# k2-fsa/Flow2GAN

Measured on AMD Instinct MI355X. Metric: audio-seconds/sec (train step, G+D fwd/bwd) mel_24k_base, higher is better.
Workload: dtype f32 (fp32-class products on the bf16 matrix pipe for the long reductions and the direct MRD convs: every fp32 operand as three bf16 pieces = 24 significand bits, the six v_mfma_f32_32x32x16_bf16 products with i + j <= 2 per fp32 product, fp32 accumulate, error <= 2^-23 per product; short reductions ; 1 GPU; mel_24k_base GAN stage-2 train step: D-step + G-step, each on its own batch (MPD+MRD+FM+multi-scale mel), fwd+bwd+grad all-reduce, no optimizer (metric is fwd/bwd); per_gpu_batch=64, gan=gan_multi_scale_mel_recon, parallelism=dp1, optimizer=none

## Files before the change

flow2gan_amd/csrc/conv32x6.hip:

```cpp
#include <stdlib.h>

#include "common.h"


namespace {

typedef float f32x16 __attribute__((ext_vector_type(16)));
typedef float f32x4 __attribute__((ext_vector_type(4)));
typedef __bf16 bf16x8 __attribute__((ext_vector_type(8)));
typedef unsigned int u32x2 __attribute__((ext_vector_type(2)));
typedef unsigned int u32x4 __attribute__((ext_vector_type(4)));

constexpr int C = 32, KH = 3, KW = 9, NTAP = KH * KW;
constexpr int PB = 208;

__device__ __attribute__((aligned(16))) float c6_zero[4] = {0.f, 0.f, 0.f, 0.f};

__device__ __forceinline__ void split3(const f32x4 v, u32x2& p0, u32x2& p1, u32x2& p2) {
  unsigned a0, a1, a2, b0, b1, b2;
  f2g_split3_pair(v.x, v.y, a0, a1, a2);
  f2g_split3_pair(v.z, v.w, b0, b1, b2);
  p0 = u32x2{a0, b0};
  p1 = u32x2{a1, b1};
  p2 = u32x2{a2, b2};
}

__device__ __forceinline__ void store_px3(unsigned char* p, const f32x4 v) {
  u32x2 p0, p1, p2;
  split3(v, p0, p1, p2);
  *reinterpret_cast<u32x2*>(p) = p0;
  *reinterpret_cast<u32x2*>(p + 64) = p1;
  *reinterpret_cast<u32x2*>(p + 128) = p2;
}

struct frag6 {
  bf16x8 v[2][3];
};
__device__ __forceinline__ void ld6(frag6& f, const unsigned char* p) {
#pragma unroll
  for (int ks = 0; ks < 2; ++ks)
#pragma unroll
    for (int q = 0; q < 3; ++q) f.v[ks][q] = *reinterpret_cast<const bf16x8*>(p + q * 64 + ks * 32);
}
__device__ __forceinline__ void mm6(const frag6& a, const frag6& b, f32x16& acc0, f32x16& acc1) {
#define F2G_X6_PAIR(I, J)                                                               \
  acc0 = __builtin_amdgcn_mfma_f32_32x32x16_bf16(a.v[0][I], b.v[0][J], acc0, 0, 0, 0);   \
  acc1 = __builtin_amdgcn_mfma_f32_32x32x16_bf16(a.v[1][I], b.v[1][J], acc1, 0, 0, 0);
  F2G_X6_PAIR(2, 0) F2G_X6_PAIR(1, 1) F2G_X6_PAIR(0, 2) F2G_X6_PAIR(1, 0) F2G_X6_PAIR(0, 1) F2G_X6_PAIR(0, 0)
#undef F2G_X6_PAIR
}
__device__ __forceinline__ void tap6(const unsigned char* Ab, const unsigned char* Bb, f32x16& acc0, f32x16& acc1) {
  frag6 a, b;
  ld6(a, Ab);
  ld6(b, Bb);
  mm6(a, b, acc0, acc1);
}

template <int D>
__device__ __forceinline__ int div_small(int x) {
  static_assert(D == 39 || D == 23 || D == 20 || D == 12, "magic constants below");
  return (x * (D == 39 ? 1681 : D == 23 ? 2850 : D == 20 ? 3277 : 5462)) >> 16;
}

template <int TW_>
__device__ __forceinline__ void px_of_row(int pg, int r, int& ph, int& pw) {
  if (TW_ == 16) {
    ph = 2 * pg + (r >> 4);
    pw = (r + 12 * (r >> 4)) & 15;
  } else {
    const int p = pg * 32 + r;
    ph = p / TW_;
    pw = p % TW_;
  }
}

template <int TH_, int TW_>
__global__ __launch_bounds__(512, 1) void conv32_s2_fwd6_kernel(const f2g_conv32_desc d, int tiles_w,
                                                               int tiles_h, int ntiles) {
  constexpr int IHv = TH_ + KH - 1, IWv = TW_ + (KW - 1) / 2, XW = 2 * IWv - 1;
  constexpr int SUBB = IHv * IWv * PB + 64;
  constexpr int NCHK = (IHv * XW * (C / 4) + 511) / 512;
  constexpr int PGB = (TW_ == 16 ? 2 : 4) * IWv * PB;
  constexpr int NKS = 2 * NTAP, KPW = 7;
  static_assert(TH_ * TW_ == 128, "a block owns 128 output pixels");
  static_assert(6 * KPW + 2 * (KPW - 1) == NKS, "the k split covers the reduction exactly");
  extern __shared__ __attribute__((aligned(16))) unsigned char smb[];
  unsigned char* At = smb;
  float* red = reinterpret_cast<float*>(smb + 2 * SUBB);
  const int tid = threadIdx.x, lane = tid & 63;
  const int wave = __builtin_amdgcn_readfirstlane(tid >> 6);
  const int li = lane & 31, hh = lane >> 5;
  const int c4 = tid & 7;
  const int px0 = tid >> 3;
  auto tile_pos = [&](int tile, int& sq, int& h0, int& w0) {
    const int tw = tile % tiles_w, rest = tile / tiles_w;
    const int th = rest % tiles_h;
    sq = rest / tiles_h;
    h0 = th * TH_;
    w0 = tw * TW_;
  };
  auto load_patch = [&](int tile, f32x4 (&pf)[NCHK]) {
    int sq, h0, w0;
    tile_pos(tile, sq, h0, w0);
    const int x0 = 2 * w0 - (KW - 1) / 2;
    const float* org = d.x + (long long)sq * d.x_seq + (long long)(h0 - 1) * d.x_line + (long long)x0 * C + c4 * 4;
    const int xl = (int)d.x_line;
    int pxb = px0;
    asm volatile("" : "+v"(pxb));
#pragma unroll
    for (int q = 0; q < NCHK; ++q) {
      const int px = pxb + 64 * q;
      const int r = div_small<XW>(px), xr = px - r * XW;
      const int h = h0 - 1 + r, x = x0 + xr;
      const bool ok = px < IHv * XW && h >= 0 && h < d.H && x >= 0 && x < d.Win;
      pf[q] = *reinterpret_cast<const f32x4*>(ok ? org + (r * xl + xr * C) : c6_zero);
    }
  };
  auto store_patch = [&](const f32x4 (&pf)[NCHK]) {
    int pxb = px0;
    asm volatile("" : "+v"(pxb));
#pragma unroll
    for (int q = 0; q < NCHK; ++q) {
      const int px = pxb + 64 * q;
      const int r = div_small<XW>(px), xr = px - r * XW;
      if (px < IHv * XW) store_px3(At + (xr & 1) * SUBB + (r * IWv + (xr >> 1)) * PB + c4 * 8, pf[q]);
    }
  };
  int tile = blockIdx.x;
  if (tile >= ntiles) return;
  f32x4 pf[NCHK];
  load_patch(tile, pf);
  const int k0 = wave * KPW - (wave == 7 ? 1 : 0);
  const bool seven = wave < 6;
  bf16x8 wf[KPW][3];
  int koff[KPW];
  {
    const unsigned char* wrow = reinterpret_cast<const unsigned char*>(d.w) + li * (NTAP * 192) + hh * 16;
#pragma unroll
    for (int j = 0; j < KPW; ++j) {
      int k = k0 + j;
      k = k < NKS ? k : NKS - 1;
      const int t = k >> 1, ks = k & 1;
      const int dh = t / KW, jw = t - dh * KW;
      koff[j] = (jw & 1) * SUBB + (dh * IWv + (jw >> 1)) * PB + ks * 32;
#pragma unroll
      for (int q = 0; q < 3; ++q) wf[j][q] = *reinterpret_cast<const bf16x8*>(wrow + t * 192 + q * 64 + ks * 32);
    }
  }
  int ph, pw;
  px_of_row<TW_>(0, li, ph, pw);
  const unsigned char* Ap = At + (ph * IWv + pw) * PB + hh * 16;
  const int orow = (wave & 3) * 8 + (lane >> 3), och = 4 * (lane & 7);
  f32x4 bias4 = {0.f, 0.f, 0.f, 0.f};
  if (d.bias) bias4 = f32x4{d.bias[och], d.bias[och + 1], d.bias[och + 2], d.bias[och + 3]};
  store_patch(pf);
  __syncthreads();
  for (; tile < ntiles; tile += gridDim.x) {
    const int nxt = tile + gridDim.x;
    const bool more = nxt < ntiles;
    load_patch(more ? nxt : tile, pf);
    f32x16 acc[4];
#pragma unroll
    for (int g4 = 0; g4 < 4; ++g4)
#pragma unroll
      for (int e = 0; e < 16; ++e) acc[g4][e] = 0.f;
    bf16x8 a[2][3];
#pragma unroll
    for (int q = 0; q < 3; ++q) a[0][q] = *reinterpret_cast<const bf16x8*>(Ap + koff[0] + q * 64);
#pragma unroll
    for (int u = 0; u < 4 * KPW; ++u) {
      const int j = u >> 2, g4 = u & 3;
      if (u + 1 < 4 * KPW) {
        const unsigned char* an = Ap + koff[(u + 1) >> 2] + ((u + 1) & 3) * PGB;
#pragma unroll
        for (int q = 0; q < 3; ++q) a[(u + 1) & 1][q] = *reinterpret_cast<const bf16x8*>(an + q * 64);
      }
      __builtin_amdgcn_sched_barrier(0);
      if (j < KPW - 1 || seven) {
#define F2G_X6_ONE(I, J) acc[g4] = __builtin_amdgcn_mfma_f32_32x32x16_bf16(a[u & 1][I], wf[j][J], acc[g4], 0, 0, 0);
        F2G_X6_ONE(2, 0) F2G_X6_ONE(1, 1) F2G_X6_ONE(0, 2) F2G_X6_ONE(1, 0) F2G_X6_ONE(0, 1) F2G_X6_ONE(0, 0)
#undef F2G_X6_ONE
      }
      __builtin_amdgcn_sched_barrier(0);
    }
    int sq, h0, w0;
    tile_pos(tile, sq, h0, w0);
    float* ys = d.y + (long long)sq * d.y_seq;
    __syncthreads();
#pragma unroll
    for (int p2 = 0; p2 < 2; ++p2) {
      if (p2) __syncthreads();
#pragma unroll
      for (int g2 = 0; g2 < 2; ++g2)
#pragma unroll
        for (int e = 0; e < 16; ++e)
          red[((wave * 2 + g2) * 32 + (e & 3) + 8 * (e >> 2) + 4 * hh) * 32 + li] = acc[2 * p2 + g2][e];
      __syncthreads();
      f32x4 s = *reinterpret_cast<const f32x4*>(red + (((wave >> 2)) * 32 + orow) * 32 + och);
#pragma unroll
      for (int w8 = 1; w8 < 8; ++w8) {
        const f32x4 v = *reinterpret_cast<const f32x4*>(red + ((w8 * 2 + (wave >> 2)) * 32 + orow) * 32 + och);
        s.x += v.x, s.y += v.y, s.z += v.z, s.w += v.w;
      }
      s.x += bias4.x, s.y += bias4.y, s.z += bias4.z, s.w += bias4.w;
      if (d.lrelu_slope != 0.f) {
        s.x = s.x > 0.f ? s.x : d.lrelu_slope * s.x;
        s.y = s.y > 0.f ? s.y : d.lrelu_slope * s.y;
        s.z = s.z > 0.f ? s.z : d.lrelu_slope * s.z;
        s.w = s.w > 0.f ? s.w : d.lrelu_slope * s.w;
      }
      int qh, qw;
      px_of_row<TW_>(2 * p2 + (wave >> 2), orow, qh, qw);
      const int oh = h0 + qh, ow = w0 + qw;
      if (oh < d.H && ow < d.Wout)
        *reinterpret_cast<f32x4*>(ys + (long long)oh * d.y_line + (long long)ow * C + och) = s;
      if (p2 == 0 && more) store_patch(pf);
    }
  }
}

template <int TH_, int TW_>
__global__ __launch_bounds__(512, 1) void conv32_s2_dgrad6_kernel(const f2g_conv32_desc d, int tiles_w,
                                                                 int tiles_h, int ntiles) {
  constexpr int IHv = TH_ + KH - 1, GWv = TW_ + 4;
  constexpr int NCHK = (IHv * GWv * (C / 4) + 511) / 512;
  constexpr int PGB = (TW_ == 16 ? 2 : 4) * GWv * PB;
  constexpr int KPW = 8;
  static_assert(TH_ * TW_ == 128, "a block owns 128 positions of each column parity");
  extern __shared__ __attribute__((aligned(16))) unsigned char smb[];
  unsigned char* At = smb;
  float* red = reinterpret_cast<float*>(smb + IHv * GWv * PB);
  const int tid = threadIdx.x, lane = tid & 63;
  const int wave = __builtin_amdgcn_readfirstlane(tid >> 6);
  const int li = lane & 31, hh = lane >> 5;
  const int wq = wave & 3, E = wave >> 2;
  const int c4 = tid & 7;
  const int NU = E ? 4 : 5;
  const int Wp = (d.Win + 1 - E) / 2;
  const int px0 = tid >> 3;
  auto tile_pos = [&](int tile, int& sq, int& h0, int& m0) {
    const int tw = tile % tiles_w, rest = tile / tiles_w;
    const int th = rest % tiles_h;
    sq = rest / tiles_h;
    h0 = th * TH_;
    m0 = tw * TW_;
  };
  auto load_patch = [&](int tile, f32x4 (&pf)[NCHK]) {
    int sq, h0, m0;
    tile_pos(tile, sq, h0, m0);
    const float* org = d.x + (long long)sq * d.x_seq + (long long)(h0 - 1) * d.x_line + (long long)(m0 - 2) * C + c4 * 4;
    const int xl = (int)d.x_line;
    int pxb = px0;
    asm volatile("" : "+v"(pxb));
#pragma unroll
    for (int q = 0; q < NCHK; ++q) {
      const int px = pxb + 64 * q;
      const int r = div_small<GWv>(px), xc = px - r * GWv;
      const int h = h0 - 1 + r, c = m0 - 2 + xc;
      const bool ok = px < IHv * GWv && h >= 0 && h < d.H && c >= 0 && c < d.Wout;
      pf[q] = *reinterpret_cast<const f32x4*>(ok ? org + (r * xl + xc * C) : c6_zero);
    }
  };
  auto store_patch = [&](const f32x4 (&pf)[NCHK]) {
#pragma unroll
    for (int q = 0; q < NCHK; ++q) {
      const int px = px0 + 64 * q;
      if (px < IHv * GWv) store_px3(At + px * PB + c4 * 8, pf[q]);
    }
  };
  int tile = blockIdx.x;
  if (tile >= ntiles) return;
  f32x4 pf[NCHK];
  load_patch(tile, pf);
  const int nk = E ? 6 : (wq < 2 ? 8 : 7);
  const int k0 = E ? 6 * wq : (wq < 2 ? 8 * wq : 16 + 7 * (wq - 2));
  bf16x8 wf[KPW][3];
  int koff[KPW];
  {
    const unsigned char* wrow = reinterpret_cast<const unsigned char*>(d.w) + li * 192 + hh * 16;
    const int nks = 2 * KH * NU;
#pragma unroll
    for (int j = 0; j < KPW; ++j) {
      int k = k0 + j;
      k = k < nks ? k : nks - 1;
      const int ti = k >> 1, ks = k & 1;
      const int dh = E ? ti >> 2 : (ti * 13) >> 6;
      const int u = ti - dh * NU;
      koff[j] = ks * 32 - (dh * GWv + u) * PB;
      const int tile_w = dh * KW + E + 2 * u;
#pragma unroll
      for (int q = 0; q < 3; ++q)
        wf[j][q] = *reinterpret_cast<const bf16x8*>(wrow + tile_w * (C * 192) + q * 64 + ks * 32);
    }
  }
  int ph, pw;
  px_of_row<TW_>(0, li, ph, pw);
  const unsigned char* Ap = At + ((ph + 2) * GWv + pw + 4) * PB + hh * 16;
  const int och = 4 * (lane & 7);
  const bool msk = d.mask_src != nullptr, fm = d.fm_ref != nullptr;
  const float fmw = fm ? d.fm_w * (d.fm_wdev ? d.fm_wdev[0] : 1.f) : 0.f;
  float cs[4] = {0.f, 0.f, 0.f, 0.f};
  store_patch(pf);
  __syncthreads();
  for (; tile < ntiles; tile += gridDim.x) {
    const int nxt = tile + gridDim.x;
    const bool more = nxt < ntiles;
    load_patch(more ? nxt : tile, pf);
    int sq, h0, m0;
    tile_pos(tile, sq, h0, m0);
    const long long tbase = (long long)sq * d.y_seq + (long long)h0 * d.y_line + (long long)(2 * m0 + E) * C;
    auto item_off = [&](int jj) {
      int qh, qw, l8 = lane >> 3;
      asm volatile("" : "+v"(l8));
      px_of_row<TW_>(2 * (jj >> 1) + (wq >> 1), (wq & 1) * 16 + l8 + 8 * (jj & 1), qh, qw);
      return (h0 + qh < d.H && m0 + qw < Wp) ? qh * (int)d.y_line + 2 * qw * C + och : -1;
    };
    f32x4 my[4];
    if (msk && !fm) {
#pragma unroll
      for (int jj = 0; jj < 4; ++jj) {
        const int o = item_off(jj);
        my[jj] = *reinterpret_cast<const f32x4*>(d.mask_src + (o >= 0 ? tbase + o : 0));
      }
    }
    f32x16 acc[4];
#pragma unroll
    for (int g4 = 0; g4 < 4; ++g4)
#pragma unroll
      for (int e = 0; e < 16; ++e) acc[g4][e] = 0.f;
    bf16x8 a[2][3];
#pragma unroll
    for (int q = 0; q < 3; ++q) a[0][q] = *reinterpret_cast<const bf16x8*>(Ap + koff[0] + q * 64);
#pragma unroll
    for (int u = 0; u < 4 * KPW; ++u) {
      const int j = u >> 2, g4 = u & 3;
      if (u + 1 < 4 * KPW) {
        const unsigned char* an = Ap + koff[(u + 1) >> 2] + ((u + 1) & 3) * PGB;
#pragma unroll
        for (int q = 0; q < 3; ++q) a[(u + 1) & 1][q] = *reinterpret_cast<const bf16x8*>(an + q * 64);
      }
      __builtin_amdgcn_sched_barrier(0);
      if (j < 6 || j < nk) {
#define F2G_X6_ONE(I, J) acc[g4] = __builtin_amdgcn_mfma_f32_32x32x16_bf16(a[u & 1][I], wf[j][J], acc[g4], 0, 0, 0);
        F2G_X6_ONE(2, 0) F2G_X6_ONE(1, 1) F2G_X6_ONE(0, 2) F2G_X6_ONE(1, 0) F2G_X6_ONE(0, 1) F2G_X6_ONE(0, 0)
#undef F2G_X6_ONE
      }
      __builtin_amdgcn_sched_barrier(0);
    }
    __syncthreads();
#pragma unroll
    for (int p2 = 0; p2 < 2; ++p2) {
      if (p2) __syncthreads();
      f32x4 fv[2];
      if (msk && fm) {
#pragma unroll
        for (int i2 = 0; i2 < 2; ++i2) {
          const int o = item_off(2 * p2 + i2);
          const long long oo = o >= 0 ? tbase + o : 0;
          my[2 * p2 + i2] = *reinterpret_cast<const f32x4*>(d.mask_src + oo);
          fv[i2] = *reinterpret_cast<const f32x4*>(d.fm_ref + oo);
        }
      }
#pragma unroll
      for (int g2 = 0; g2 < 2; ++g2)
#pragma unroll
        for (int e = 0; e < 16; ++e)
          red[((wave * 2 + g2) * 32 + (e & 3) + 8 * (e >> 2) + 4 * hh) * 32 + li] = acc[2 * p2 + g2][e];
      __syncthreads();
#pragma unroll
      for (int i2 = 0; i2 < 2; ++i2) {
        const int jj = 2 * p2 + i2;
        const float* rp = red + (((E * 4) * 2 + (wq >> 1)) * 32 + (wq & 1) * 16 + (lane >> 3) + 8 * i2) * 32 + och;
        f32x4 s = *reinterpret_cast<const f32x4*>(rp);
#pragma unroll
        for (int w4 = 1; w4 < 4; ++w4) {
          const f32x4 v = *reinterpret_cast<const f32x4*>(rp + w4 * (2 * 32 * 32));
          s.x += v.x, s.y += v.y, s.z += v.z, s.w += v.w;
        }
        const int o = item_off(jj);
        if (o < 0) continue;
        float v[4] = {s.x, s.y, s.z, s.w};
        if (msk && !fm) {
          const float y[4] = {my[jj].x, my[jj].y, my[jj].z, my[jj].w};
#pragma unroll
          for (int e = 0; e < 4; ++e) v[e] *= y[e] > 0.f ? 1.f : d.mask_slope;
        } else if (msk) {
          const float y[4] = {my[jj].x, my[jj].y, my[jj].z, my[jj].w}, f[4] = {fv[i2].x, fv[i2].y, fv[i2].z, fv[i2].w};
#pragma unroll
          for (int e = 0; e < 4; ++e) {
            const float dl = y[e] - f[e];
            v[e] += fmw * (dl > 0.f ? 1.f : (dl < 0.f ? -1.f : 0.f));
            v[e] *= y[e] > 0.f ? 1.f : d.mask_slope;
          }
        }
#pragma unroll
        for (int e = 0; e < 4; ++e) cs[e] += v[e];
        *reinterpret_cast<f32x4*>(d.y + tbase + o) = f32x4{v[0], v[1], v[2], v[3]};
      }
      if (p2 == 0 && more) store_patch(pf);
    }
  }
  if (d.colsum) {
    float* csl = reinterpret_cast<float*>(At);
#pragma unroll
    for (int e = 0; e < 4; ++e) {
      float v = cs[e];
      v += __shfl_xor(v, 8);
      v += __shfl_xor(v, 16);
      v += __shfl_xor(v, 32);
      if (lane < 8) csl[wave * 32 + 4 * lane + e] = v;
    }
    __syncthreads();
    if (tid < 32) {
      float v = csl[tid];
#pragma unroll
      for (int w8 = 1; w8 < 8; ++w8) v += csl[w8 * 32 + tid];
      atomicAdd(d.colsum + tid, v);
    }
  }
}

typedef short s16x4 __attribute__((ext_vector_type(4)));
constexpr int GPL = 128 * 64;
constexpr int GCH = 128 * (C / 4) / 512;

__device__ __forceinline__ bf16x8 tr_pix8(const unsigned char* p) {
  typedef s16x4 __attribute__((address_space(3))) * lds_p;
  const s16x4 a = __builtin_amdgcn_ds_read_tr16_b64_v4i16((lds_p)(p));
  const s16x4 b = __builtin_amdgcn_ds_read_tr16_b64_v4i16((lds_p)(p + 4 * 64));
  return __builtin_bit_cast(bf16x8, __builtin_shufflevector(a, b, 0, 1, 2, 3, 4, 5, 6, 7));
}

template <int TH, int TW>
__global__ __launch_bounds__(512, 1) void conv32_s2_wgrad6_kernel(const f2g_conv32_desc d, float* gw,
                                                                  int tiles_h, int tiles_w,
                                                                  int tiles_per_block) {
  constexpr int IH = TH + KH - 1, IW = TW + (KW - 1) / 2, XW = 2 * IW - 1;
  constexpr int XPAR = IH * IW * 64 + 64;
  constexpr int XPL = 2 * XPAR;
  constexpr int XCH = (IH * XW * (C / 4) + 511) / 512;
  constexpr int KR = 16 / TW;
  constexpr int NK = TH / KR;
  static_assert(TH * TW == 128 && NK == 8 && XCH <= NK && GCH <= NK, "tile shapes");
  extern __shared__ __attribute__((aligned(16))) unsigned char smb[];
  unsigned char* Xp = smb;
  unsigned char* Gp = smb + 3 * XPL;
  const int tid = threadIdx.x, lane = tid & 63, wave = tid >> 6;
  const int li = lane & 31, hh = lane >> 5;
  const int ntiles = d.S * tiles_h * tiles_w;
  f32x16 acc[6];
#pragma unroll
  for (int a = 0; a < 6; ++a)
#pragma unroll
    for (int e = 0; e < 16; ++e) acc[a][e] = 0.f;
  const int g4 = lane >> 4, i16 = lane & 15;
  const int kpix = (g4 >> 1) * 8 + (i16 >> 2);
  const int kpat = TW == 16 ? kpix : (g4 >> 1) * IW + (i16 >> 2);
  const int chb = (g4 & 1) * 32 + (i16 & 3) * 8;
  int xo[3], xs[3];
#pragma unroll
  for (int a = 0; a < 3; ++a) {
    int t = wave + 8 * a;
    int dh = t / KW, j = t - dh * KW;
    xo[a] = (j & 1) * XPAR + (dh * IW + (j >> 1) + kpat) * 64 + chb;
    t = 24 + a;
    dh = t / KW;
    j = t - dh * KW;
    xs[a] = (j & 1) * XPAR + (dh * IW + (j >> 1) + kpat) * 64 + chb;
  }
  const int go = kpix * 64 + chb;
  const int c4 = tid & 7, px0 = tid >> 3;
  auto xoff = [&](int q) {
    const int px = px0 + 64 * q;
    const int r = div_small<XW>(px), xr = px - r * XW;
    return px < IH * XW ? (xr & 1) * XPAR + (r * IW + (xr >> 1)) * 64 + c4 * 8 : -1;
  };
  auto tile_pos = [&](int ti, int& s, int& h0, int& w0) {
    s = ti / (tiles_h * tiles_w);
    const int rem = ti - s * (tiles_h * tiles_w);
    const int th = rem / tiles_w;
    h0 = th * TH;
    w0 = (rem - th * tiles_w) * TW;
  };
// ... 313 lines not shown
        split3(px_[q], pk[0], pk[1], pk[2]);
#pragma unroll
        for (int pc = 0; pc < 3; ++pc) *reinterpret_cast<u32x2*>(Xp + pc * W33_XPL + (px + 1) * 64 + c4 * 8) = pk[pc];
      }
      if (grow[q] > -(1 << 21)) {
        split3(pg_[q], pk[0], pk[1], pk[2]);
#pragma unroll
        for (int pc = 0; pc < 3; ++pc) *reinterpret_cast<u32x2*>(Gp + pc * W33_GPL + px * 64 + c4 * 8) = pk[pc];
      }
    }
    __syncthreads();
    for (int ks = wave; ks < nks; ks += 8) {
      bf16x8 a[3];
#pragma unroll
      for (int q = 0; q < 3; ++q) a[q] = tr_pix8(Gp + q * W33_GPL + ks * (16 * 64) + go);
#pragma unroll
      for (int t = 0; t < T33; ++t) {
        bf16x8 b[3];
#pragma unroll
        for (int q = 0; q < 3; ++q) b[q] = tr_pix8(Xp + q * W33_XPL + ks * (16 * 64) + xo[t]);
        mfma6(a, b, acc[t]);
      }
    }
    __syncthreads();
  }
  float* red = reinterpret_cast<float*>(smb);
#pragma unroll
  for (int t = 0; t < T33; ++t) {
    __syncthreads();
#pragma unroll
    for (int e = 0; e < 16; ++e) red[(wave * 16 + e) * 64 + lane] = acc[t][e];
    __syncthreads();
    if (wave == (t & 7)) {
#pragma unroll
      for (int e = 0; e < 16; ++e) {
        float v = 0.f;
#pragma unroll
        for (int w8 = 0; w8 < 8; ++w8) v += red[(w8 * 16 + e) * 64 + lane];
        const int co = (e & 3) + 8 * (e >> 2) + 4 * hh;
        atomicAdd(gw + co * (T33 * C) + t * C + li, v);
      }
    }
  }
}

template <int TH_, int TW_>
constexpr size_t fwd6_smem() {
  return (size_t)2 * ((TH_ + 2) * (TW_ + 4) * PB + 64) + 8 * 2 * 32 * 32 * sizeof(float);
}
template <int TH_, int TW_>
constexpr size_t dgrad6_smem() {
  return (size_t)(TH_ + 2) * (TW_ + 4) * PB + 8 * 2 * 32 * 32 * sizeof(float);
}

}

int f2g_conv32_fwd6_launch(const f2g_conv32_desc* d, hipStream_t st) {
  auto waste = [&](int th, int tw) {
    return (long long)((d->H + th - 1) / th * th) * ((d->Wout + tw - 1) / tw * tw);
  };
  const bool tall = waste(16, 8) < waste(8, 16);
  const int th = tall ? 16 : 8, tw = tall ? 8 : 16;
  const int tiles_h = (d->H + th - 1) / th, tiles_w = (d->Wout + tw - 1) / tw;
  const long long nt = (long long)tiles_h * tiles_w * d->S;
  if (nt >= (1ll << 30) || d->x_line >= (1ll << 24)) return F2G_EINVAL;
  static bool attr = false;
  if (!attr) {
    (void)hipFuncSetAttribute(reinterpret_cast<const void*>(conv32_s2_fwd6_kernel<8, 16>),
                              hipFuncAttributeMaxDynamicSharedMemorySize, (int)(fwd6_smem<8, 16>()));
    (void)hipFuncSetAttribute(reinterpret_cast<const void*>(conv32_s2_fwd6_kernel<16, 8>),
                              hipFuncAttributeMaxDynamicSharedMemorySize, (int)(fwd6_smem<16, 8>()));
    attr = true;
  }
  const int grid = (int)(nt < 256 ? nt : 256);
  if (tall)
    hipLaunchKernelGGL((conv32_s2_fwd6_kernel<16, 8>), dim3(grid), dim3(512), (fwd6_smem<16, 8>()), st, *d,
                       tiles_w, tiles_h, (int)nt);
  else
    hipLaunchKernelGGL((conv32_s2_fwd6_kernel<8, 16>), dim3(grid), dim3(512), (fwd6_smem<8, 16>()), st, *d,
                       tiles_w, tiles_h, (int)nt);
  return f2g_check_launch();
}

int f2g_conv32_dgrad6_launch(const f2g_conv32_desc* d, hipStream_t st) {
  const int Wp0 = (d->Win + 1) / 2;
  auto waste = [&](int th, int tw) {
    return (long long)((d->H + th - 1) / th * th) * ((Wp0 + tw - 1) / tw * tw);
  };
  const bool tall = waste(16, 8) < waste(8, 16);
  const int th = tall ? 16 : 8, tw = tall ? 8 : 16;
  const int tiles_h = (d->H + th - 1) / th, tiles_w = (Wp0 + tw - 1) / tw;
  const long long nt = (long long)tiles_h * tiles_w * d->S;
  if (nt >= (1ll << 30) || d->x_line >= (1ll << 24) || d->y_line >= (1ll << 24)) return F2G_EINVAL;
  static bool attr = false;
  if (!attr) {
    (void)hipFuncSetAttribute(reinterpret_cast<const void*>(conv32_s2_dgrad6_kernel<8, 16>),
                              hipFuncAttributeMaxDynamicSharedMemorySize, (int)(dgrad6_smem<8, 16>()));
    (void)hipFuncSetAttribute(reinterpret_cast<const void*>(conv32_s2_dgrad6_kernel<16, 8>),
                              hipFuncAttributeMaxDynamicSharedMemorySize, (int)(dgrad6_smem<16, 8>()));
    attr = true;
  }
  const int grid = (int)(nt < 256 ? nt : 256);
  if (tall)
    hipLaunchKernelGGL((conv32_s2_dgrad6_kernel<16, 8>), dim3(grid), dim3(512), (dgrad6_smem<16, 8>()), st, *d,
                       tiles_w, tiles_h, (int)nt);
  else
    hipLaunchKernelGGL((conv32_s2_dgrad6_kernel<8, 16>), dim3(grid), dim3(512), (dgrad6_smem<8, 16>()), st, *d,
                       tiles_w, tiles_h, (int)nt);
  return f2g_check_launch();
}

int f2g_conv32_wgrad6_launch(const f2g_conv32_desc* d, float* gw, hipStream_t st) {
  auto waste = [&](int th, int tw) {
    return (long long)((d->H + th - 1) / th * th) * ((d->Wout + tw - 1) / tw * tw);
  };
  const bool tall = waste(16, 8) < waste(8, 16);
  const int th = tall ? 16 : 8, tw = tall ? 8 : 16;
  const int tiles_h = (d->H + th - 1) / th, tiles_w = (d->Wout + tw - 1) / tw;
  const long long nt = (long long)d->S * tiles_h * tiles_w;
  if (nt >= (1ll << 30) || d->x_line >= (1ll << 24)) return F2G_EINVAL;
  int per = (int)((nt + 255) / 256);
  if (per < 1) per = 1;
  constexpr size_t sm8 = (size_t)3 * 2 * ((8 + 2) * (16 + 4) * 64 + 64) + 3 * GPL;
  constexpr size_t sm16 = (size_t)3 * 2 * ((16 + 2) * (8 + 4) * 64 + 64) + 3 * GPL;
  static_assert(sm8 >= (size_t)8 * 16 * 64 * 4 && sm16 >= (size_t)8 * 16 * 64 * 4,
                "the flush reuses the planes as its reduction buffer");
  static bool attr = false;
  if (!attr) {
    (void)hipFuncSetAttribute(reinterpret_cast<const void*>(conv32_s2_wgrad6_kernel<8, 16>),
                              hipFuncAttributeMaxDynamicSharedMemorySize, (int)sm8);
    (void)hipFuncSetAttribute(reinterpret_cast<const void*>(conv32_s2_wgrad6_kernel<16, 8>),
                              hipFuncAttributeMaxDynamicSharedMemorySize, (int)sm16);
    attr = true;
  }
  const unsigned grid = (unsigned)((nt + per - 1) / per);
  if (tall)
    hipLaunchKernelGGL((conv32_s2_wgrad6_kernel<16, 8>), dim3(grid), dim3(512), sm16, st, *d, gw, tiles_h, tiles_w, per);
  else
    hipLaunchKernelGGL((conv32_s2_wgrad6_kernel<8, 16>), dim3(grid), dim3(512), sm8, st, *d, gw, tiles_h, tiles_w, per);
  return f2g_check_launch();
}

extern "C" int f2g_conv33_fwd(const f2g_conv32_desc* d, f2g_stream_t stream) {
  if (!d || !d->x || !d->w || !d->y || d->precision != 3 || d->Win != d->Wout || d->fm_ref) return F2G_EINVAL;
  if ((((uintptr_t)d->x) & 15) || (((uintptr_t)d->w) & 15) || (d->x_line & 3) || (d->x_seq & 3)) return F2G_EINVAL;
  if (d->S <= 0 || d->H <= 0 || d->Win <= 0) return F2G_OK;
  const int W = d->Win;
  if (W > 112 || d->x_line >= (1ll << 24)) return F2G_EINVAL;
  if (d->y_line < (long long)W * C || (d->y != d->x && d->y_seq < (long long)d->H * d->y_line)) return F2G_EINVAL;
  if ((d->y_line & 3) || (d->y_seq & 3) || (((uintptr_t)d->y) & 15)) return F2G_EINVAL;
  if (d->mask_src && (d->lrelu_slope != 0.f || d->bias || (((uintptr_t)d->mask_src) & 15))) {
    f2g_set_error("f2g_conv33_fwd: mask_src (data-gradient role) excludes bias / lrelu_slope (forward role)");
    return F2G_EINVAL;
  }
  int R = 256 / W;
  if (R > d->H) R = d->H;
  while (R > 1 && (R + 2) * (W + 2) > P33) --R;
  if (R < 1 || (R + 2) * (W + 2) > P33) return F2G_EINVAL;
  const int tiles_h = (d->H + R - 1) / R;
  const long long nt = (long long)tiles_h * d->S;
  if (nt >= (1ll << 30)) return F2G_EINVAL;
  constexpr size_t smem = (size_t)P33 * PB + (size_t)T33 * C * PB;
  static bool attr = false;
  if (!attr) {
    (void)hipFuncSetAttribute(reinterpret_cast<const void*>(conv33_x6_kernel),
                              hipFuncAttributeMaxDynamicSharedMemorySize, (int)smem);
    attr = true;
  }
  const int grid = (int)(nt < 256 ? nt : 256);
  hipLaunchKernelGGL(conv33_x6_kernel, dim3(grid), dim3(512), smem, (hipStream_t)stream, *d, R, tiles_h, (int)nt);
  return f2g_check_launch();
}

extern "C" int f2g_conv33_wgrad(const f2g_conv32_desc* d, float* gw, f2g_stream_t stream) {
  if (!d || !d->x || !d->y || !gw || d->precision != 3 || d->Win != d->Wout) return F2G_EINVAL;
  if ((((uintptr_t)d->x) & 15) || (((uintptr_t)d->y) & 15) || (d->x_line & 3) || (d->x_seq & 3) || (d->y_line & 3) ||
      (d->y_seq & 3))
    return F2G_EINVAL;
  if (d->S <= 0 || d->H <= 0 || d->Win <= 0) return F2G_OK;
  const int W = d->Win;
  if (W > 112 || d->x_line >= (1ll << 24) || d->y_line >= (1ll << 24) || d->x_line < (long long)W * C ||
      d->y_line < (long long)W * C)
    return F2G_EINVAL;
  int R = 256 / W;
  if (R > d->H) R = d->H;
  while (R > 1 && (R + 2) * (W + 2) > P33) --R;
  if (R < 1 || (R + 2) * (W + 2) > P33) return F2G_EINVAL;
  const int tiles_h = (d->H + R - 1) / R;
  const long long nt = (long long)tiles_h * d->S;
  if (nt >= (1ll << 30)) return F2G_EINVAL;
  constexpr size_t smem = (size_t)3 * (W33_XPL + W33_GPL);
// ... 14 lines not shown
```

Baseline: 811.6 audio-s/s.

## Pipeline MRD conv32 fwd/dgrad epilogue reductions with next pixel group's MFMAs

Restructures the fwd6 and dgrad6 stride-2 conv kernels. Each wave now holds a single 32x32 accumulator per pixel group instead of four, and writes it to a double-buffered LDS reduction area. The cross-wave reduction and epilogue (bias, leaky ReLU, mask and feature-matching terms, store) of the previous group, including the last group of the previous tile, are interleaved with the current group's MFMA chain. The bf16 three-way split of the prefetched next patch is also spread across MFMA slots using sched_group_barrier, and dgrad gains an EPI template parameter so the mask/FM branches are resolved at compile time. The aim is to hide barrier, reduction and split latency behind matrix work and to lower register pressure, at the cost of more complex scheduling and a remapped TW=8 pixel rotation that must stay consistent between the producer and reduction layouts.

```diff
diff --git a/flow2gan_amd/csrc/conv32x6.hip b/flow2gan_amd/csrc/conv32x6.hip
--- a/flow2gan_amd/csrc/conv32x6.hip
+++ b/flow2gan_amd/csrc/conv32x6.hip
@@ -33,6 +33,19 @@
   *reinterpret_cast<u32x2*>(p + 128) = p2;
 }
 
+__device__ __forceinline__ void split3_now(const f32x4 v, u32x2 (&pk)[3]) {
+  split3(v, pk[0], pk[1], pk[2]);
+#pragma unroll
+  for (int q = 0; q < 3; ++q) asm volatile("" : "+v"(pk[q].x), "+v"(pk[q].y));
+}
+__device__ __forceinline__ void store_pk3(unsigned char* p, const u32x2 (&pk)[3]) {
+  *reinterpret_cast<u32x2*>(p) = pk[0];
+  *reinterpret_cast<u32x2*>(p + 64) = pk[1];
+  *reinterpret_cast<u32x2*>(p + 128) = pk[2];
+}
+
+__device__ __forceinline__ void c6_barrier() { asm volatile("s_waitcnt lgkmcnt(0)\n\ts_barrier" ::: "memory"); }
+
 struct frag6 {
   bf16x8 v[2][3];
 };
@@ -64,13 +77,14 @@
 
 template <int TW_>
 __device__ __forceinline__ void px_of_row(int pg, int r, int& ph, int& pw) {
+  static_assert(TW_ == 16 || TW_ == 8, "the rotations are worked out for these row widths");
   if (TW_ == 16) {
     ph = 2 * pg + (r >> 4);
     pw = (r + 12 * (r >> 4)) & 15;
   } else {
-    const int p = pg * 32 + r;
-    ph = p / TW_;
-    pw = p % TW_;
+    const int row = r >> 3;
+    ph = pg * 4 + row;
+    pw = (r + 4 * (((row + 1) >> 1) & 1)) & 7;
   }
 }
 
@@ -116,14 +130,14 @@
       pf[q] = *reinterpret_cast<const f32x4*>(ok ? org + (r * xl + xr * C) : c6_zero);
     }
   };
-  auto store_patch = [&](const f32x4 (&pf)[NCHK]) {
+  auto store_pieces = [&](const u32x2 (&pk)[NCHK][3]) {
     int pxb = px0;
     asm volatile("" : "+v"(pxb));
 #pragma unroll
     for (int q = 0; q < NCHK; ++q) {
       const int px = pxb + 64 * q;
       const int r = div_small<XW>(px), xr = px - r * XW;
-      if (px < IHv * XW) store_px3(At + (xr & 1) * SUBB + (r * IWv + (xr >> 1)) * PB + c4 * 8, pf[q]);
+      if (px < IHv * XW) store_pk3(At + (xr & 1) * SUBB + (r * IWv + (xr >> 1)) * PB + c4 * 8, pk[q]);
     }
   };
   int tile = blockIdx.x;
@@ -151,75 +165,112 @@
   px_of_row<TW_>(0, li, ph, pw);
   const unsigned char* Ap = At + (ph * IWv + pw) * PB + hh * 16;
   const int orow = (wave & 3) * 8 + (lane >> 3), och = 4 * (lane & 7);
+  const int ohalf = wave >> 2;
   f32x4 bias4 = {0.f, 0.f, 0.f, 0.f};
   if (d.bias) bias4 = f32x4{d.bias[och], d.bias[och + 1], d.bias[och + 2], d.bias[och + 3]};
-  store_patch(pf);
-  __syncthreads();
+  auto red_item = [&](int g, int w8) {
+    return *reinterpret_cast<const f32x4*>(red + (((g & 1) * 8 + w8) * 32 + orow) * 32 + och);
+  };
+  auto finish = [&](f32x4 s, float* ys, int h0, int w0, int g) {
+    s.x += bias4.x, s.y += bias4.y, s.z += bias4.z, s.w += bias4.w;
+    if (d.lrelu_slope != 0.f) {
+      s.x = s.x > 0.f ? s.x : d.lrelu_slope * s.x;
+      s.y = s.y > 0.f ? s.y : d.lrelu_slope * s.y;
+      s.z = s.z > 0.f ? s.z : d.lrelu_slope * s.z;
+      s.w = s.w > 0.f ? s.w : d.lrelu_slope * s.w;
+    }
+    int qh, qw;
+    px_of_row<TW_>(g, orow, qh, qw);
+    const int oh = h0 + qh, ow = w0 + qw;
+    if (oh < d.H && ow < d.Wout)
+      *reinterpret_cast<f32x4*>(ys + (long long)oh * d.y_line + (long long)ow * C + och) = s;
+  };
+  u32x2 pk[NCHK][3];
+#pragma unroll
+  for (int q = 0; q < NCHK; ++q) split3(pf[q], pk[q][0], pk[q][1], pk[q][2]);
+  store_pieces(pk);
+  c6_barrier();
+  __builtin_amdgcn_s_waitcnt(0x0F70);
+  float* pys = d.y;
+  int ph0 = 0, pw0 = 0;
+  bool prev = false;
   for (; tile < ntiles; tile += gridDim.x) {
     const int nxt = tile + gridDim.x;
     const bool more = nxt < ntiles;
     load_patch(more ? nxt : tile, pf);
-    f32x16 acc[4];
-#pragma unroll
-    for (int g4 = 0; g4 < 4; ++g4)
-#pragma unroll
-      for (int e = 0; e < 16; ++e) acc[g4][e] = 0.f;
-    bf16x8 a[2][3];
-#pragma unroll
-    for (int q = 0; q < 3; ++q) a[0][q] = *reinterpret_cast<const bf16x8*>(Ap + koff[0] + q * 64);
-#pragma unroll
-    for (int u = 0; u < 4 * KPW; ++u) {
-      const int j = u >> 2, g4 = u & 3;
-      if (u + 1 < 4 * KPW) {
-        const unsigned char* an = Ap + koff[(u + 1) >> 2] + ((u + 1) & 3) * PGB;
-#pragma unroll
-        for (int q = 0; q < 3; ++q) a[(u + 1) & 1][q] = *reinterpret_cast<const bf16x8*>(an + q * 64);
-      }
-      __builtin_amdgcn_sched_barrier(0);
-      if (j < KPW - 1 || seven) {
-#define F2G_X6_ONE(I, J) acc[g4] = __builtin_amdgcn_mfma_f32_32x32x16_bf16(a[u & 1][I], wf[j][J], acc[g4], 0, 0, 0);
-        F2G_X6_ONE(2, 0) F2G_X6_ONE(1, 1) F2G_X6_ONE(0, 2) F2G_X6_ONE(1, 0) F2G_X6_ONE(0, 1) F2G_X6_ONE(0, 0)
-#undef F2G_X6_ONE
-      }
-      __builtin_amdgcn_sched_barrier(0);
-    }
     int sq, h0, w0;
     tile_pos(tile, sq, h0, w0);
     float* ys = d.y + (long long)sq * d.y_seq;
-    __syncthreads();
-#pragma unroll
-    for (int p2 = 0; p2 < 2; ++p2) {
-      if (p2) __syncthreads();
-#pragma unroll
-      for (int g2 = 0; g2 < 2; ++g2)
-#pragma unroll
-        for (int e = 0; e < 16; ++e)
-          red[((wave * 2 + g2) * 32 + (e & 3) + 8 * (e >> 2) + 4 * hh) * 32 + li] = acc[2 * p2 + g2][e];
-      __syncthreads();
-      f32x4 s = *reinterpret_cast<const f32x4*>(red + (((wave >> 2)) * 32 + orow) * 32 + och);
-#pragma unroll
-      for (int w8 = 1; w8 < 8; ++w8) {
-        const f32x4 v = *reinterpret_cast<const f32x4*>(red + ((w8 * 2 + (wave >> 2)) * 32 + orow) * 32 + och);
-        s.x += v.x, s.y += v.y, s.z += v.z, s.w += v.w;
-      }
-      s.x += bias4.x, s.y += bias4.y, s.z += bias4.z, s.w += bias4.w;
-      if (d.lrelu_slope != 0.f) {
-        s.x = s.x > 0.f ? s.x : d.lrelu_slope * s.x;
-        s.y = s.y > 0.f ? s.y : d.lrelu_slope * s.y;
-        s.z = s.z > 0.f ? s.z : d.lrelu_slope * s.z;
-        s.w = s.w > 0.f ? s.w : d.lrelu_slope * s.w;
-      }
-      int qh, qw;
-      px_of_row<TW_>(2 * p2 + (wave >> 2), orow, qh, qw);
-      const int oh = h0 + qh, ow = w0 + qw;
-      if (oh < d.H && ow < d.Wout)
-        *reinterpret_cast<f32x4*>(ys + (long long)oh * d.y_line + (long long)ow * C + och) = s;
-      if (p2 == 0 && more) store_patch(pf);
-    }
-  }
-}
-
-template <int TH_, int TW_>
+    f32x16 acc;
+    bf16x8 a[2][3];
+    f32x4 s = {0.f, 0.f, 0.f, 0.f}, rv0 = s, rv1 = s;
+#pragma unroll
+    for (int q = 0; q < 3; ++q) a[0][q] = *reinterpret_cast<const bf16x8*>(Ap + koff[0] + q * 64);
+#pragma unroll
+    for (int u = 0; u < 4 * KPW; ++u) {
+      const int q = u / KPW, j = u % KPW;
+      if (j == 0) {
+#pragma unroll
+        for (int e = 0; e < 16; ++e) acc[e] = 0.f;
+      }
+      const int og = (q + 3) & 3;
+      if (ohalf == (og & 1) && (q > 0 || prev)) {
+        if (j == 1) s = rv0;
+        if (j > 1 && j <= 4) s.x += rv0.x, s.y += rv0.y, s.z += rv0.z, s.w += rv0.w;
+        if (j >= 1 && j <= 4) s.x += rv1.x, s.y += rv1.y, s.z += rv1.z, s.w += rv1.w;
+        if (j < 4) {
+          rv0 = red_item(og, 2 * j);
+          rv1 = red_item(og, 2 * j + 1);
+        }
+        if (j == 4) finish(s, q ? ys : pys, q ? h0 : ph0, q ? w0 : pw0, og);
+      }
+      __builtin_amdgcn_sched_barrier(0);
+      if (u + 1 < 4 * KPW) {
+        const unsigned char* an = Ap + koff[(u + 1) % KPW] + ((u + 1) / KPW) * PGB;
+#pragma unroll
+        for (int q3 = 0; q3 < 3; ++q3) a[(u + 1) & 1][q3] = *reinterpret_cast<const bf16x8*>(an + q3 * 64);
+      }
+      if (q == 3 && j < NCHK) split3_now(pf[j], pk[j]);
+      else __builtin_amdgcn_sched_barrier(0);
+      if (j < KPW - 1 || seven) {
+#define F2G_X6_ONE(I, J) acc = __builtin_amdgcn_mfma_f32_32x32x16_bf16(a[u & 1][I], wf[j][J], acc, 0, 0, 0);
+        F2G_X6_ONE(2, 0) F2G_X6_ONE(1, 1) F2G_X6_ONE(0, 2) F2G_X6_ONE(1, 0) F2G_X6_ONE(0, 1) F2G_X6_ONE(0, 0)
+#undef F2G_X6_ONE
+      }
+      if (q == 3 && j < KPW - 1) {
+        __builtin_amdgcn_sched_group_barrier(0x100, 3, 0);
+#pragma unroll
+        for (int m = 0; m < 6; ++m) {
+          __builtin_amdgcn_sched_group_barrier(0x008, 1, 0);
+          __builtin_amdgcn_sched_group_barrier(0x002, 4, 0);
+        }
+      }
+      __builtin_amdgcn_sched_barrier(0);
+      if (j == KPW - 1) {
+        float* wp = red + ((q & 1) * 8 + wave) * (32 * 32) + li;
+#pragma unroll
+        for (int e = 0; e < 16; ++e) wp[((e & 3) + 8 * (e >> 2) + 4 * hh) * 32] = acc[e];
+        c6_barrier();
+      }
+    }
+    if (more) {
+      store_pieces(pk);
+      c6_barrier();
+    }
+    pys = ys, ph0 = h0, pw0 = w0, prev = true;
+  }
+  if (ohalf == 1) {
+    f32x4 s = red_item(3, 0);
+#pragma unroll
+    for (int w8 = 1; w8 < 8; ++w8) {
+      const f32x4 v = red_item(3, w8);
+      s.x += v.x, s.y += v.y, s.z += v.z, s.w += v.w;
+    }
+    finish(s, pys, ph0, pw0, 3);
+  }
+}
+
+template <int TH_, int TW_, int EPI>
 __global__ __launch_bounds__(512, 1) void conv32_s2_dgrad6_kernel(const f2g_conv32_desc d, int tiles_w,
                                                                  int tiles_h, int ntiles) {
   constexpr int IHv = TH_ + KH - 1, GWv = TW_ + 4;
@@ -261,11 +312,11 @@
       pf[q] = *reinterpret_cast<const f32x4*>(ok ? org + (r * xl + xc * C) : c6_zero);
     }
   };
-  auto store_patch = [&](const f32x4 (&pf)[NCHK]) {
+  auto store_pieces = [&](const u32x2 (&pk)[NCHK][3]) {
 #pragma unroll
     for (int q = 0; q < NCHK; ++q) {
       const int px = px0 + 64 * q;
-      if (px < IHv * GWv) store_px3(At + px * PB + c4 * 8, pf[q]);
+      if (px < IHv * GWv) store_pk3(At + px * PB + c4 * 8, pk[q]);
     }
   };
   int tile = blockIdx.x;
@@ -296,12 +347,49 @@
   int ph, pw;
   px_of_row<TW_>(0, li, ph, pw);
   const unsigned char* Ap = At + ((ph + 2) * GWv + pw + 4) * PB + hh * 16;
-  const int och = 4 * (lane & 7);
-  const bool msk = d.mask_src != nullptr, fm = d.fm_ref != nullptr;
+  const int opos = wq * 8 + (lane >> 3), och = 4 * (lane & 7);
+  constexpr bool msk = EPI >= 1, fm = EPI == 2;
   const float fmw = fm ? d.fm_w * (d.fm_wdev ? d.fm_wdev[0] : 1.f) : 0.f;
   float cs[4] = {0.f, 0.f, 0.f, 0.f};
-  store_patch(pf);
-  __syncthreads();
+  auto red_item = [&](int g, int w4) {
+    return *reinterpret_cast<const f32x4*>(red + (((g & 1) * 8 + E * 4 + w4) * 32 + opos) * 32 + och);
+  };
+  auto item_off = [&](int g, int h0, int m0) {
+    int qh, qw;
+    px_of_row<TW_>(g, opos, qh, qw);
+    return (h0 + qh < d.H && m0 + qw < Wp) ? qh * (int)d.y_line + 2 * qw * C + och : -1;
+  };
+  auto finish = [&](const f32x4 s, long long base, int o, const f32x4 y4, const f32x4 f4) {
+    if (o < 0) return;
+    float v[4] = {s.x, s.y, s.z, s.w};
+    if (msk && !fm) {
+      const float y[4] = {y4.x, y4.y, y4.z, y4.w};
+#pragma unroll
+      for (int e = 0; e < 4; ++e) v[e] *= y[e] > 0.f ? 1.f : d.mask_slope;
+    } else if (msk) {
+      const float y[4] = {y4.x, y4.y, y4.z, y4.w}, f[4] = {f4.x, f4.y, f4.z, f4.w};
+#pragma unroll
+      for (int e = 0; e < 4; ++e) {
+        const float dl = y[e] - f[e];
+        v[e] += fmw * (dl > 0.f ? 1.f : (dl < 0.f ? -1.f : 0.f));
+        v[e] *= y[e] > 0.f ? 1.f : d.mask_slope;
+      }
+    }
+#pragma unroll
+    for (int e = 0; e < 4; ++e) cs[e] += v[e];
+    *reinterpret_cast<f32x4*>(d.y + base + o) = f32x4{v[0], v[1], v[2], v[3]};
+  };
+  u32x2 pk[NCHK][3];
+#pragma unroll
+  for (int q = 0; q < NCHK; ++q) split3(pf[q], pk[q][0], pk[q][1], pk[q][2]);
+  store_pieces(pk);
+  c6_barrier();
+  __builtin_amdgcn_s_waitcnt(0x0F70);
+  long long pbase = 0;
+  bool prev = false;
+  f32x4 my[2], fv[2];
+  int io[2] = {-1, -1};
+  my[0] = my[1] = fv[0] = fv[1] = f32x4{0.f, 0.f, 0.f, 0.f};
   for (; tile < ntiles; tile += gridDim.x) {
     const int nxt = tile + gridDim.x;
     const bool more = nxt < ntiles;
@@ -309,96 +397,83 @@
     int sq, h0, m0;
     tile_pos(tile, sq, h0, m0);
     const long long tbase = (long long)sq * d.y_seq + (long long)h0 * d.y_line + (long long)(2 * m0 + E) * C;
-    auto item_off = [&](int jj) {
-      int qh, qw, l8 = lane >> 3;
-      asm volatile("" : "+v"(l8));
-      px_of_row<TW_>(2 * (jj >> 1) + (wq >> 1), (wq & 1) * 16 + l8 + 8 * (jj & 1), qh, qw);
-      return (h0 + qh < d.H && m0 + qw < Wp) ? qh * (int)d.y_line + 2 * qw * C + och : -1;
-    };
-    f32x4 my[4];
-    if (msk && !fm) {
-#pragma unroll
-      for (int jj = 0; jj < 4; ++jj) {
-        const int o = item_off(jj);
-        my[jj] = *reinterpret_cast<const f32x4*>(d.mask_src + (o >= 0 ? tbase + o : 0));
-      }
-    }
-    f32x16 acc[4];
-#pragma unroll
-    for (int g4 = 0; g4 < 4; ++g4)
-#pragma unroll
-      for (int e = 0; e < 16; ++e) acc[g4][e] = 0.f;
+    f32x16 acc;
     bf16x8 a[2][3];
+    f32x4 s = {0.f, 0.f, 0.f, 0.f}, rv0 = s, rv1 = s;
 #pragma unroll
     for (int q = 0; q < 3; ++q) a[0][q] = *reinterpret_cast<const bf16x8*>(Ap + koff[0] + q * 64);
 #pragma unroll
     for (int u = 0; u < 4 * KPW; ++u) {
-      const int j = u >> 2, g4 = u & 3;
+      const int q = u / KPW, j = u % KPW;
+      const int og = (q + 3) & 3;
+      if (j == 0) {
+#pragma unroll
+        for (int e = 0; e < 16; ++e) acc[e] = 0.f;
+        const int o = item_off(q, h0, m0);
+        const long long oo = o >= 0 ? tbase + o : 0;
+        io[q & 1] = o;
+        if (msk) my[q & 1] = *reinterpret_cast<const f32x4*>(d.mask_src + oo);
+        if (msk && fm) fv[q & 1] = *reinterpret_cast<const f32x4*>(d.fm_ref + oo);
+      }
+      if (q > 0 || prev) {
+        if (j == 0) {
+          rv0 = red_item(og, 0);
+          rv1 = red_item(og, 1);
+        }
+        if (j == 1) {
+          s = f32x4{rv0.x + rv1.x, rv0.y + rv1.y, rv0.z + rv1.z, rv0.w + rv1.w};
+          rv0 = red_item(og, 2);
+          rv1 = red_item(og, 3);
+        }
+        if (j == 2) {
+          s.x += rv0.x, s.y += rv0.y, s.z += rv0.z, s.w += rv0.w;
+          s.x += rv1.x, s.y += rv1.y, s.z += rv1.z, s.w += rv1.w;
+          finish(s, q ? tbase : pbase, io[og & 1], my[og & 1], fv[og & 1]);
+        }
+      }
+      __builtin_amdgcn_sched_barrier(0);
       if (u + 1 < 4 * KPW) {
-        const unsigned char* an = Ap + koff[(u + 1) >> 2] + ((u + 1) & 3) * PGB;
-#pragma unroll
-        for (int q = 0; q < 3; ++q) a[(u + 1) & 1][q] = *reinterpret_cast<const bf16x8*>(an + q * 64);
-      }
-      __builtin_amdgcn_sched_barrier(0);
+        const unsigned char* an = Ap + koff[(u + 1) % KPW] + ((u + 1) / KPW) * PGB;
+#pragma unroll
+        for (int q3 = 0; q3 < 3; ++q3) a[(u + 1) & 1][q3] = *reinterpret_cast<const bf16x8*>(an + q3 * 64);
+      }
+      if (q == 3 && j < NCHK) split3_now(pf[j], pk[j]);
+      else __builtin_amdgcn_sched_barrier(0);
       if (j < 6 || j < nk) {
-#define F2G_X6_ONE(I, J) acc[g4] = __builtin_amdgcn_mfma_f32_32x32x16_bf16(a[u & 1][I], wf[j][J], acc[g4], 0, 0, 0);
+#define F2G_X6_ONE(I, J) acc = __builtin_amdgcn_mfma_f32_32x32x16_bf16(a[u & 1][I], wf[j][J], acc, 0, 0, 0);
         F2G_X6_ONE(2, 0) F2G_X6_ONE(1, 1) F2G_X6_ONE(0, 2) F2G_X6_ONE(1, 0) F2G_X6_ONE(0, 1) F2G_X6_ONE(0, 0)
 #undef F2G_X6_ONE
       }
+      if (q == 3 && j < NCHK) {
+        __builtin_amdgcn_sched_group_barrier(0x100, 3, 0);
+#pragma unroll
+        for (int m = 0; m < 6; ++m) {
+          __builtin_amdgcn_sched_group_barrier(0x008, 1, 0);
+          __builtin_amdgcn_sched_group_barrier(0x002, 4, 0);
+        }
+      }
       __builtin_amdgcn_sched_barrier(0);
-    }
-    __syncthreads();
-#pragma unroll
-    for (int p2 = 0; p2 < 2; ++p2) {
-      if (p2) __syncthreads();
-      f32x4 fv[2];
-      if (msk && fm) {
-#pragma unroll
-        for (int i2 = 0; i2 < 2; ++i2) {
-          const int o = item_off(2 * p2 + i2);
-          const long long oo = o >= 0 ? tbase + o : 0;
-          my[2 * p2 + i2] = *reinterpret_cast<const f32x4*>(d.mask_src + oo);
-          fv[i2] = *reinterpret_cast<const f32x4*>(d.fm_ref + oo);
-        }
-      }
-#pragma unroll
-      for (int g2 = 0; g2 < 2; ++g2)
-#pragma unroll
-        for (int e = 0; e < 16; ++e)
-          red[((wave * 2 + g2) * 32 + (e & 3) + 8 * (e >> 2) + 4 * hh) * 32 + li] = acc[2 * p2 + g2][e];
-      __syncthreads();
-#pragma unroll
-      for (int i2 = 0; i2 < 2; ++i2) {
-        const int jj = 2 * p2 + i2;
-        const float* rp = red + (((E * 4) * 2 + (wq >> 1)) * 32 + (wq & 1) * 16 + (lane >> 3) + 8 * i2) * 32 + och;
-        f32x4 s = *reinterpret_cast<const f32x4*>(rp);
-#pragma unroll
-        for (int w4 = 1; w4 < 4; ++w4) {
-          const f32x4 v = *reinterpret_cast<const f32x4*>(rp + w4 * (2 * 32 * 32));
-          s.x += v.x, s.y += v.y, s.z += v.z, s.w += v.w;
-        }
-        const int o = item_off(jj);
-        if (o < 0) continue;
-        float v[4] = {s.x, s.y, s.z, s.w};
-        if (msk && !fm) {
-          const float y[4] = {my[jj].x, my[jj].y, my[jj].z, my[jj].w};
-#pragma unroll
-          for (int e = 0; e < 4; ++e) v[e] *= y[e] > 0.f ? 1.f : d.mask_slope;
-        } else if (msk) {
-          const float y[4] = {my[jj].x, my[jj].y, my[jj].z, my[jj].w}, f[4] = {fv[i2].x, fv[i2].y, fv[i2].z, fv[i2].w};
-#pragma unroll
-          for (int e = 0; e < 4; ++e) {
-            const float dl = y[e] - f[e];
-            v[e] += fmw * (dl > 0.f ? 1.f : (dl < 0.f ? -1.f : 0.f));
-            v[e] *= y[e] > 0.f ? 1.f : d.mask_slope;
-          }
-        }
-#pragma unroll
-        for (int e = 0; e < 4; ++e) cs[e] += v[e];
-        *reinterpret_cast<f32x4*>(d.y + tbase + o) = f32x4{v[0], v[1], v[2], v[3]};
-      }
-      if (p2 == 0 && more) store_patch(pf);
-    }
+      if (j == KPW - 1) {
+        float* wp = red + ((q & 1) * 8 + wave) * (32 * 32) + li;
+#pragma unroll
+        for (int e = 0; e < 16; ++e) wp[((e & 3) + 8 * (e >> 2) + 4 * hh) * 32] = acc[e];
+        c6_barrier();
+      }
+    }
+    if (more) {
+      store_pieces(pk);
+      c6_barrier();
+    }
+    pbase = tbase, prev = true;
+  }
+  {
+    f32x4 s = red_item(3, 0);
+#pragma unroll
+    for (int w4 = 1; w4 < 4; ++w4) {
+      const f32x4 v = red_item(3, w4);
+      s.x += v.x, s.y += v.y, s.z += v.z, s.w += v.w;
+    }
+    finish(s, pbase, io[1], my[1], fv[1]);
   }
   if (d.colsum) {
     float* csl = reinterpret_cast<float*>(At);
@@ -878,6 +953,18 @@
   return f2g_check_launch();
 }
 
+template <int TH_, int TW_, int EPI>
+static void dgrad6_go(const f2g_conv32_desc* d, int grid, int tiles_w, int tiles_h, int nt, hipStream_t st) {
+  static bool attr = false;
+  if (!attr) {
+    (void)hipFuncSetAttribute(reinterpret_cast<const void*>(conv32_s2_dgrad6_kernel<TH_, TW_, EPI>),
+                              hipFuncAttributeMaxDynamicSharedMemorySize, (int)(dgrad6_smem<TH_, TW_>()));
+    attr = true;
+  }
+  hipLaunchKernelGGL((conv32_s2_dgrad6_kernel<TH_, TW_, EPI>), dim3(grid), dim3(512), (dgrad6_smem<TH_, TW_>()), st,
+                     *d, tiles_w, tiles_h, nt);
+}
+
 int f2g_conv32_dgrad6_launch(const f2g_conv32_desc* d, hipStream_t st) {
   const int Wp0 = (d->Win + 1) / 2;
   auto waste = [&](int th, int tw) {
@@ -888,21 +975,17 @@
   const int tiles_h = (d->H + th - 1) / th, tiles_w = (Wp0 + tw - 1) / tw;
   const long long nt = (long long)tiles_h * tiles_w * d->S;
   if (nt >= (1ll << 30) || d->x_line >= (1ll << 24) || d->y_line >= (1ll << 24)) return F2G_EINVAL;
-  static bool attr = false;
-  if (!attr) {
-    (void)hipFuncSetAttribute(reinterpret_cast<const void*>(conv32_s2_dgrad6_kernel<8, 16>),
-                              hipFuncAttributeMaxDynamicSharedMemorySize, (int)(dgrad6_smem<8, 16>()));
-    (void)hipFuncSetAttribute(reinterpret_cast<const void*>(conv32_s2_dgrad6_kernel<16, 8>),
-                              hipFuncAttributeMaxDynamicSharedMemorySize, (int)(dgrad6_smem<16, 8>()));
-    attr = true;
-  }
   const int grid = (int)(nt < 256 ? nt : 256);
-  if (tall)
-    hipLaunchKernelGGL((conv32_s2_dgrad6_kernel<16, 8>), dim3(grid), dim3(512), (dgrad6_smem<16, 8>()), st, *d,
-                       tiles_w, tiles_h, (int)nt);
-  else
-    hipLaunchKernelGGL((conv32_s2_dgrad6_kernel<8, 16>), dim3(grid), dim3(512), (dgrad6_smem<8, 16>()), st, *d,
-                       tiles_w, tiles_h, (int)nt);
+  const int epi = d->mask_src ? (d->fm_ref ? 2 : 1) : 0;
+  if (tall) {
+    if (epi == 0) dgrad6_go<16, 8, 0>(d, grid, tiles_w, tiles_h, (int)nt, st);
+    else if (epi == 1) dgrad6_go<16, 8, 1>(d, grid, tiles_w, tiles_h, (int)nt, st);
+    else dgrad6_go<16, 8, 2>(d, grid, tiles_w, tiles_h, (int)nt, st);
+  } else {
+    if (epi == 0) dgrad6_go<8, 16, 0>(d, grid, tiles_w, tiles_h, (int)nt, st);
+    else if (epi == 1) dgrad6_go<8, 16, 1>(d, grid, tiles_w, tiles_h, (int)nt, st);
+    else dgrad6_go<8, 16, 2>(d, grid, tiles_w, tiles_h, (int)nt, st);
+  }
   return f2g_check_launch();
 }
 
```

After: 817.7 audio-s/s (median of 4 runs). Within noise of the previous version (+0.7%).
